# lliutianc/MPVAE-1

Measured on AMD Instinct MI355X. Metric: probit MC label-samples/sec (B×n_sample×L) at 1/2/4/8 GPU; ELBO rel-err, higher is better.
Workload: dtype f32; 1 GPU; c4: compute_loss fwd+bwd, B=512, L=1024, z=1024, n_sample=4096 (4096/GPU), philox noise on device; global_batch=512, n_sample=4096, label_dim=1024, z_dim=1024, parallelism=n_sample-sharded x1, gemm=f16x3

## Files before the change

### mpvae-1_amd/csrc/probit_fwd.hip

```cpp
#include <cstdlib>
#include <cstring>

#include "abi_util.h"
#include "mpv_common.h"

namespace mpv {

int launch_sum_slabs(const float* in, int64_t nslab, int64_t n, void* out, int out_dtype,
                     hipStream_t s);

struct FwdParams {
  const float* y;
  const float* fe;
  const float* fx;
  const float* R;
  const float* eps;
  mpv_split16 R16;
  mpv_split16 eps16;
  float* T;
  float* rowpart;
  float* colpart;
  int S, B, L, z;
  int ldT;
  int nNt, nSc, tps, nSt;
// ... 350 lines not shown
#pragma unroll
      for (int kk = 0; kk < kBK / 16; ++kk) {
        f32x4 a[TM], bb[TN];
#pragma unroll
        for (int m = 0; m < TM; ++m)
          a[m] = *reinterpret_cast<const f32x4*>(
              &As[(wm * TM * 16 + m * 16 + lr) * kLDK + kk * 16 + lg * 4]);
#pragma unroll
        for (int n = 0; n < TN; ++n)
          bb[n] = *reinterpret_cast<const f32x4*>(
              &Bs[(wn * TN * 16 + n * 16 + lr) * kLDK + kk * 16 + lg * 4]);
#pragma unroll
        for (int j = 0; j < 4; ++j)
#pragma unroll
          for (int m = 0; m < TM; ++m)
#pragma unroll
            for (int n = 0; n < TN; ++n)
              acc[m][n] = __builtin_amdgcn_mfma_f32_16x16x4f32(a[m][j], bb[n][j], acc[m][n], 0, 0, 0);
      }
      __syncthreads();
      if (kc + 1 < nK) {
        store_tiles();
        __syncthreads();
      }
    }
    if constexpr (PREDICT)
      fwd_tile_epilogue_predict<WM, WN, TM, TN>(p, ln, acc, 1.0f, b, s0, s0, nt);
    else
      fwd_tile_epilogue<WM, WN, TM, TN>(p, ln, acc, 1.0f, b, s0, s0, nt, smem);
  }
  fwd_colsum_epilogue<WM, WN, TM, TN, PREDICT>(p, ln, b, sc, n0, smem);
}

constexpr int kKC = 32;
constexpr int kRowB = 128;
constexpr int kFwdRing = 2;
constexpr int kFwd16Threads = 512;

template <int BM>
MPV_DEV int fwd_tile_s0(int st, int S) {
  return S >= BM ? min(st * BM, S - BM) : 0;
}

template <int BM, int BN, int NW>
struct Fwd16Dma {
  static constexpr int GA = BM / 8, GB = BN / 8;
  static constexpr int JA = (GA + NW - 1) / NW, JB = (GB + NW - 1) / NW;
  const char* a_base;
  const char* b_base;
  uint32_t offa[JA], offb[JB];
  int tile, kc;
  int wid;

  MPV_DEV void init(const FwdParams& p, int t0, int b, int n0, int wid_, int lane) {
    wid = wid_;
    const int64_t lda = p.eps16.ld, ldb = p.R16.ld;
    const int prow = lane >> 3, u_lds = lane & 7;
    b_base = reinterpret_cast<const char*>(p.R16.data + (int64_t)n0 * ldb);
#pragma unroll
    for (int j = 0; j < JA; ++j) {
      const int r = (wid + j * NW) * 8 + prow;
      offa[j] = (uint32_t)((int64_t)min(r, p.S - 1) * lda * 2) +
                (uint32_t)((u_lds ^ ((r >> 1) & 7)) * 16);
    }
#pragma unroll
    for (int j = 0; j < JB; ++j) {
      const int r = (wid + j * NW) * 8 + prow;
      offb[j] = (uint32_t)(r * ldb * 2) + (uint32_t)((u_lds ^ ((r >> 1) & 7)) * 16);
    }
    tile = t0;
    kc = 0;
    set_tile(p, b);
  }

  MPV_DEV void set_tile(const FwdParams& p, int b) {
    const int64_t o = ((int64_t)b * p.S + fwd_tile_s0<BM>(tile, p.S)) * p.eps16.ld;
    a_base = reinterpret_cast<const char*>(p.eps16.data + o);
  }

  MPV_DEV static void piece(const char* base, uint32_t off, char* dst) {
    lds_dma16(base, off, lds_addr(dst));
  }

  MPV_DEV void issue(const FwdParams& p, char* dst, int tile_end, int nK, int b) {
    if (tile >= tile_end) return;
    const int kb = kc * kRowB;
#pragma unroll
    for (int j = 0; j < JA; ++j) {
      const int pc = wid + j * NW;
      if (GA % NW == 0 || pc < GA) piece(a_base + kb, offa[j], dst + pc * 1024);
    }
#pragma unroll
    for (int j = 0; j < JB; ++j) {
      const int pc = wid + j * NW;
      if (GB % NW == 0 || pc < GB) piece(b_base + kb, offb[j], dst + BM * kRowB + pc * 1024);
    }
    if (++kc == nK) {
      kc = 0;
      if (++tile < tile_end) set_tile(p, b);
    }
  }
};

template <int BM, int BN, int NW>
struct Fwd16DmaLin {
  static constexpr int GA = BM / 8, GB = BN / 8;
  static constexpr int JA = GA / NW, JB = GB / NW;
  static_assert(GA % NW == 0 && GB % NW == 0, "pieces split evenly over the DMA waves");
  const char* a_base;
  const char* b_base;
  int64_t a_step, b_step;
  uint32_t offa, offb;
  int tile, kc, wid;

  MPV_DEV void init(const FwdParams& p, int t0, int b, int n0, int wid_, int lane) {
    wid = wid_;
    const int64_t lda = p.eps16.ld, ldb = p.R16.ld;
    const int prow = lane >> 3, u_lds = lane & 7;
    a_step = (int64_t)NW * 8 * lda * 2;
    b_step = (int64_t)NW * 8 * ldb * 2;
    b_base = reinterpret_cast<const char*>(p.R16.data + ((int64_t)n0 + wid * 8) * ldb);
    offa = (uint32_t)(prow * lda * 2) + (uint32_t)((u_lds ^ (((wid * 8 + prow) >> 1) & 7)) * 16);
    offb = (uint32_t)(prow * ldb * 2) + (uint32_t)((u_lds ^ (((wid * 8 + prow) >> 1) & 7)) * 16);
    tile = t0;
    kc = 0;
    set_tile(p, b);
  }
  MPV_DEV void set_tile(const FwdParams& p, int b) {
    const int64_t o = ((int64_t)b * p.S + fwd_tile_s0<BM>(tile, p.S) + wid * 8) * p.eps16.ld;
    a_base = reinterpret_cast<const char*>(p.eps16.data + o);
  }
  MPV_DEV void issue(const FwdParams& p, char* dst, int tile_end, int nK, int b) {
    if (tile >= tile_end) return;
    const int kb = kc * kRowB;
#pragma unroll
    for (int j = 0; j < JA; ++j)
      lds_dma16(a_base + kb + j * a_step, offa, lds_addr(dst + (wid + j * NW) * 1024));
#pragma unroll
    for (int j = 0; j < JB; ++j)
      lds_dma16(b_base + kb + j * b_step, offb, lds_addr(dst + BM * kRowB + (wid + j * NW) * 1024));
    if (++kc == nK) {
      kc = 0;
      if (++tile < tile_end) set_tile(p, b);
    }
  }
};

struct Fwd16tTile48x256 {
  static constexpr int WL = 1, WS = 8, TL = 3, TSA = kFwd48BM / 128, TSB = TSA;
  static constexpr int BM = kFwd48BM, BN = 48, LDS_MIN = 82 * 1024;
  using Dma = Fwd16Dma<BM, BN, 4>;
  static constexpr int CQ = 1, EPI_BLOCKS = kEpiSampleBlocks, EPI_PART = 0;
  static constexpr bool RED_IN_RING = false, AHEAD = false;
};
struct Fwd16tTile96x128 {
  static constexpr int WL = 2, WS = 4, TL = 3, TSA = 2, TSB = 2;
  static constexpr int BM = 128, BN = 96, LDS_MIN = 0;
  using Dma = Fwd16Dma<BM, BN, 4>;
  static constexpr int CQ = 1, EPI_BLOCKS = kEpiSampleBlocks, EPI_PART = 0;
  static constexpr bool RED_IN_RING = false, AHEAD = false;
};
struct Fwd16aTile128x128 {
  static constexpr int WL = 4, WS = 2, TL = 2, TSA = 5, TSB = 3;
  static constexpr int BM = 128, BN = 128, LDS_MIN = 0;
  using Dma = Fwd16Dma<BM, BN, 4>;
  static constexpr int CQ = 1, EPI_BLOCKS = kEpiSampleBlocks, EPI_PART = 0;
  static constexpr bool RED_IN_RING = false, AHEAD = false;
};
struct Fwd16aTile256x128 {
  static constexpr int WL = 4, WS = 2, TL = 4, TSA = 5, TSB = 3;
  static constexpr int BM = 128, BN = 256, LDS_MIN = 0;
  using Dma = Fwd16Dma<BM, BN, 4>;
  static constexpr int CQ = 1, EPI_BLOCKS = kEpiSampleBlocks, EPI_PART = 0;
  static constexpr bool RED_IN_RING = false, AHEAD = false;
};
struct Fwd16bTile256x256 {
  static constexpr int WL = 4, WS = 2, TL = 4, TSA = kFwdBA, TSB = 16 - kFwdBA;
  static constexpr int BM = 256, BN = 256, LDS_MIN = 0;
  using Dma = Fwd16DmaLin<BM, BN, 4>;
  static constexpr int CQ = kFwdBCQ, EPI_BLOCKS = kFwdBEpi, EPI_PART = kFwdBPart;
  static constexpr bool RED_IN_RING = true, AHEAD = true;
};

template <int TL, int TS>
struct FragT {
  s16x8 rh[TL], rl[TL], eh[TS], el[TS];
};

template <int TL, int TS, int BM>
MPV_DEV void fwd16t_read(FragT<TL, TS>& f, const char* base, int wl, int sbo, int lr, int coh,
                         int col) {
#pragma unroll
  for (int m = 0; m < TL; ++m) {
    const int off = (BM + (wl * TL + m) * 16 + lr) * kRowB;
    f.rh[m] = *reinterpret_cast<const s16x8*>(base + off + coh);
    f.rl[m] = *reinterpret_cast<const s16x8*>(base + off + col);
  }
#pragma unroll
  for (int n = 0; n < TS; ++n) {
    const int off = ((sbo + n) * 16 + lr) * kRowB;
    f.eh[n] = *reinterpret_cast<const s16x8*>(base + off + coh);
    f.el[n] = *reinterpret_cast<const s16x8*>(base + off + col);
  }
}

template <int TL, int TS>
MPV_DEV void fwd16t_mfma(f32x4 (&acc)[TL][TS], const FragT<TL, TS>& f) {
#pragma unroll
  for (int m = 0; m < TL; ++m)
#pragma unroll
    for (int n = 0; n < TS; ++n)
      acc[m][n] = __builtin_amdgcn_mfma_f32_16x16x32_f16(as_f16x8(f.rh[m]), as_f16x8(f.eh[n]),
                                                         acc[m][n], 0, 0, 0);
#pragma unroll
  for (int m = 0; m < TL; ++m)
#pragma unroll
    for (int n = 0; n < TS; ++n)
      acc[m][n] = __builtin_amdgcn_mfma_f32_16x16x32_f16(as_f16x8(f.rh[m]), as_f16x8(f.el[n]),
                                                         acc[m][n], 0, 0, 0);
#pragma unroll
  for (int m = 0; m < TL; ++m)
#pragma unroll
    for (int n = 0; n < TS; ++n)
      acc[m][n] = __builtin_amdgcn_mfma_f32_16x16x32_f16(as_f16x8(f.rl[m]), as_f16x8(f.eh[n]),
                                                         acc[m][n], 0, 0, 0);
}

template <int H>
MPV_DEV f32x2 pk_fma_bc(f32x2 a, f32x2 b, f32x2 c) {
  f32x2 d;
  if (H == 0)
    asm("v_pk_fma_f32 %0, %1, %2, %3 op_sel_hi:[1,0,0]" : "=v"(d) : "v"(a), "v"(b), "v"(c));
  else
    asm("v_pk_fma_f32 %0, %1, %2, %3 op_sel:[0,1,1] op_sel_hi:[1,1,1]"
        : "=v"(d) : "v"(a), "v"(b), "v"(c));
  return d;
}
template <int H>
MPV_DEV void pk_fma2_acc_bc(f32x2 p, f32x2 q, f32x2 r, f32x2& sp, f32x2& sn) {
  if (H == 0)
    asm("s_nop 0\n\tv_pk_fma_f32 %0, %2, %4, %0 op_sel_hi:[0,1,1]\n\t"
        "v_pk_fma_f32 %1, %3, %4, %1 op_sel_hi:[0,1,1]"
        : "+v"(sp), "+v"(sn) : "v"(p), "v"(q), "v"(r));
  else
    asm("s_nop 0\n\tv_pk_fma_f32 %0, %2, %4, %0 op_sel:[1,0,0] op_sel_hi:[1,1,1]\n\t"
        "v_pk_fma_f32 %1, %3, %4, %1 op_sel:[1,0,0] op_sel_hi:[1,1,1]"
        : "+v"(sp), "+v"(sn) : "v"(p), "v"(q), "v"(r));
}

template <int BN>
MPV_DEV bool fwd_tile_soft(const FwdParams& p, int b, int n0, int nthreads) {
  bool my_soft = false;
  for (int i = threadIdx.x; i < BN; i += nthreads) {
    const int l = n0 + i;
    if (l < p.L) {
      const float yv = p.y[(int64_t)b * p.L + l];
      my_soft |= !(yv == 0.0f || yv == 1.0f);
    }
  }
  return __builtin_amdgcn_readfirstlane(__syncthreads_or(my_soft)) != 0;
}

struct Fwd16Ctx {
  int b, sc, nt, n0;
  int wid, wl, ws;
  int lr, lg;
  int coh, col;
  float scale;
  int nK;
  int t_begin, t_end;
  bool soft_any;
  float* cacc;
  const float* cols;
};

template <class Tile, bool PREDICT = false>
MPV_DEV Fwd16Ctx fwd16_ctx(const FwdParams& p, float* cacc, float* cols) {
  constexpr int WL = Tile::WL, BN = Tile::BN,
                CACC = Tile::WS * Tile::CQ * BN * (PREDICT ? 1 : 2);
  Fwd16Ctx c;
  int g;
  decode_block(blockIdx.x, p.B * p.nSc, p.nNt, g, c.nt);
  c.b = g / p.nSc, c.sc = g % p.nSc;
  c.n0 = c.nt * BN;
  const int tid = threadIdx.x, lane = tid & 63;
  c.wid = __builtin_amdgcn_readfirstlane(tid >> 6);
  c.wl = c.wid % WL, c.ws = c.wid / WL;
  c.lr = lane & 15, c.lg = lane >> 4;
  c.scale = 1.0f / (*p.eps16.scale * *p.R16.scale);
  c.nK = (p.z + kKC - 1) / kKC;
  const int sw = (c.lr >> 1) & 7;
  c.coh = (c.lg ^ sw) << 4, c.col = ((4 + c.lg) ^ sw) << 4;
  c.t_begin = c.sc * p.tps, c.t_end = min(p.nSt, (c.sc + 1) * p.tps);
  if constexpr (PREDICT)
    fwd_cols_stage_predict<BN>(cols, p, c.b, c.n0, kFwd16Threads);
  else
    fwd_cols_stage_t<BN>(cols, p, c.b, c.n0, kFwd16Threads);
  for (int i = tid; i < CACC; i += kFwd16Threads) cacc[i] = 0.0f;
  if constexpr (PREDICT)
    c.soft_any = false;
  else
    c.soft_any = fwd_tile_soft<BN>(p, c.b, c.n0, kFwd16Threads);
  c.cacc = cacc, c.cols = cols;
  return c;
}

template <class Tile, int TS, bool FIRST = true, bool LAST = true>
MPV_DEV void fwd_tile_epilogue_t(const FwdParams& p, const Fwd16Ctx c, f32x4 (&acc)[Tile::TL][TS],
                                 int s0, int s_own, int sbo, float* red) {
  constexpr int WL = Tile::WL, TL = Tile::TL, BM = Tile::BM, BN = Tile::BN, NT = kFwd16Threads;
  const int tid = threadIdx.x, lr = c.lr, lg = c.lg;
  const int wid = tid >> 6, wl = wid % WL, ws = wid / WL;
  if constexpr (Tile::TSA == Tile::TSB) {
    static_assert(TS == Tile::TSA, "the even-split tiles run the epilogue whole");
    sbo = ws * TS;
  }
  const int S = p.S, B = p.B, L = p.L, b = c.b, nt = c.nt, n0 = nt * BN;
  const float scale = c.scale;
  float* cacc = c.cacc;
  const float* cols = c.cols;
  f32x2 sl[TS], sp[TS], sn[TS];
#pragma unroll
  for (int n = 0; n < TS; ++n) sl[n] = sp[n] = sn[n] = splat2(0.0f);
#pragma unroll
  for (int m = 0; m < TL; ++m)
#pragma unroll
    for (int n = 0; n < TS; ++n) acc[m][n] = acc[m][n] * scale;
  const bool t_plain = s0 + sbo * 16 >= s_own && s0 + (sbo + TS) * 16 <= S && n0 + BN <= L;
#pragma unroll 1
  for (int m = 0; m < TL; ++m) {
    f32x4 am[TS];
#pragma unroll
    for (int n = 0; n < TS; ++n) am[n] = acc[0][n];
#pragma unroll
    for (int mm = 0; mm + 1 < TL; ++mm)
#pragma unroll
      for (int n = 0; n < TS; ++n) acc[mm][n] = acc[mm + 1][n];
    const int lb = (wl * TL + m) * 16 + lg * 4;
    if (((m + __builtin_amdgcn_readfirstlane(wid / (NT / 128))) & 1) != 0)
      __builtin_amdgcn_s_setprio(1);
    else
      __builtin_amdgcn_s_setprio(0);
    if (p.T != nullptr && t_plain) {
#pragma unroll
      for (int n = 0; n < TS; ++n) {
        const int s = s0 + (sbo + n) * 16 + lr;
        *reinterpret_cast<f32x4*>(p.T + ((int64_t)b * S + s) * p.ldT + n0 + lb) = am[n];
      }
    } else if (p.T != nullptr) {
#pragma unroll
      for (int n = 0; n < TS; ++n) {
        const int s = s0 + (sbo + n) * 16 + lr;
        if (s >= s_own && s < S) {
          float* row = p.T + ((int64_t)b * S + s) * p.ldT + n0;
          if (n0 + lb < L) {
            *reinterpret_cast<f32x4*>(row + lb) = am[n];
          } else {
#pragma unroll
            for (int i = 0; i < 4; ++i)
              if (n0 + lb + i < L) row[lb + i] = am[n][i];
          }
        }
      }
    }
    const f32x4 pa = *reinterpret_cast<const f32x4*>(cols + 2 * lb);
    const f32x4 pb = *reinterpret_cast<const f32x4*>(cols + 2 * lb + 4);
    const f32x2 fex[4] = {f32x2{pa[0], pa[1]}, f32x2{pa[2], pa[3]}, f32x2{pb[0], pb[1]},
                          f32x2{pb[2], pb[3]}};
    const f32x4 y4 = *reinterpret_cast<const f32x4*>(cols + 2 * BN + lb);
    const f32x4 qa = *reinterpret_cast<const f32x4*>(cols + kCqa * BN + lb);
    const f32x4 qb = *reinterpret_cast<const f32x4*>(cols + kCqb * BN + lb);
    const f32x4 sga = *reinterpret_cast<const f32x4*>(cols + kCsga * BN + lb);
    const f32x4 sgb = *reinterpret_cast<const f32x4*>(cols + kCsgb * BN + lb);
    const f32x4 wpos = *reinterpret_cast<const f32x4*>(cols + kCwpos * BN + lb);
    const f32x4 wneg = *reinterpret_cast<const f32x4*>(cols + kCwneg * BN + lb);
    const f32x2 qa2[2] = {f32x2{qa[0], qa[1]}, f32x2{qa[2], qa[3]}};
    const f32x2 qb2[2] = {f32x2{qb[0], qb[1]}, f32x2{qb[2], qb[3]}};
    const f32x2 sga2[2] = {f32x2{sga[0], sga[1]}, f32x2{sga[2], sga[3]}};
    const f32x2 sgb2[2] = {f32x2{sgb[0], sgb[1]}, f32x2{sgb[2], sgb[3]}};
    const f32x2 wpos2[2] = {f32x2{wpos[0], wpos[1]}, f32x2{wpos[2], wpos[3]}};
    const f32x2 wneg2[2] = {f32x2{wneg[0], wneg[1]}, f32x2{wneg[2], wneg[3]}};
    f32x2 ce[4] = {splat2(0.0f), splat2(0.0f), splat2(0.0f), splat2(0.0f)};
#pragma unroll
    for (int n = 0; n < TS; ++n) {
      const int s = s0 + (sbo + n) * 16 + lr;
      const float wr = (s >= s_own && s < S) ? 1.0f : 0.0f;
      const f32x4 t4 = am[n];
      f32x2 zq[4], w4[4];
#pragma unroll
      for (int i = 0; i < 4; ++i) zq[i] = pk_fma(splat2(t4[i]), splat2(kZq), fex[i]);
      probit_w2xN_zq<4>(zq, w4);
      f32x2 E4[4];
      {
#pragma clang fp contract(off)
#pragma unroll
        for (int i = 0; i < 4; ++i) E4[i] = w4[i] * kEh + splat2(kC0);
      }
      f32x2 q[4], r[4];
#pragma unroll
      for (int i = 0; i < 4; ++i) {
        q[i] = (i & 1) ? pk_fma_bc<1>(E4[i], qa2[i >> 1], qb2[i >> 1])
                       : pk_fma_bc<0>(E4[i], qa2[i >> 1], qb2[i >> 1]);
        const f32x2 a = (i & 1) ? pk_fma_bc<1>(E4[i], sga2[i >> 1], sgb2[i >> 1])
                                : pk_fma_bc<0>(E4[i], sga2[i >> 1], sgb2[i >> 1]);
        r[i] = f32x2{__builtin_amdgcn_exp2f(a.x), __builtin_amdgcn_exp2f(a.y)};
      }
      const f32x2 q4 = (q[0] * q[1]) * (q[2] * q[3]);
      f32x2 lp = f32x2{__builtin_amdgcn_logf(q4.x), __builtin_amdgcn_logf(q4.y)};
      if (c.soft_any) {
#pragma unroll
        for (int i = 0; i < 4; ++i) {
          const float y = y4[i];
          if (n0 + lb + i < L && !(y == 0.0f || y == 1.0f)) {
            const f32x2 E = E4[i];
            lp.x += y * __builtin_amdgcn_logf(E.x) + (1.0f - y) * __builtin_amdgcn_logf(1.0f - E.x);
            lp.y += y * __builtin_amdgcn_logf(E.y) + (1.0f - y) * __builtin_amdgcn_logf(1.0f - E.y);
          }
        }
      }
      sl[n] = sl[n] + lp;
#pragma unroll
      for (int i = 0; i < 4; ++i) {
        if (i & 1)
          pk_fma2_acc_bc<1>(wpos2[i >> 1], wneg2[i >> 1], r[i], sp[n], sn[n]);
        else
          pk_fma2_acc_bc<0>(wpos2[i >> 1], wneg2[i >> 1], r[i], sp[n], sn[n]);
        ce[i] = pk_fma(splat2(wr), E4[i], ce[i]);
      }
      if ((n + 1) % Tile::EPI_BLOCKS == 0) __builtin_amdgcn_sched_barrier(0);
    }
    float cs[8];
#pragma unroll
    for (int i = 0; i < 4; ++i) {
      cs[2 * i] = ce[i].x;
      cs[2 * i + 1] = ce[i].y;
    }
    if (Tile::CQ == 4) {
#pragma unroll
      for (int j = 0; j < 8; ++j) cs[j] = dpp_f<0x111>(cs[j]) + cs[j];
#pragma unroll
      for (int j = 0; j < 8; ++j) cs[j] = dpp_f<0x112>(cs[j]) + cs[j];
      if ((lr & 3) == 3) {
#pragma unroll
        for (int i = 0; i < 4; ++i) {
          float* c = cacc + ((ws * 4 + (lr >> 2)) * BN + lb + i) * 2;
          c[0] += cs[2 * i];
          c[1] += cs[2 * i + 1];
        }
      }
    } else {
      row16_sum_to_lane15_n<8>(cs);
      if (lr == 15) {
#pragma unroll
        for (int i = 0; i < 4; ++i) {
          float* c = cacc + (ws * BN + lb + i) * 2;
          c[0] += cs[2 * i];
          c[1] += cs[2 * i + 1];
        }
      }
    }
    __builtin_amdgcn_sched_barrier(0);
  }
  __builtin_amdgcn_sched_barrier(0);
  asm volatile("s_nop 1" ::: "memory");
  __builtin_amdgcn_sched_barrier(0);
  float v[TS * 6];
#pragma unroll
  for (int n = 0; n < TS; ++n) {
    sl[n] = sl[n] * 0.6931471805599453f;
    v[n * 6 + 0] = sl[n].x;
    v[n * 6 + 1] = sl[n].y;
    v[n * 6 + 2] = sp[n].x;
    v[n * 6 + 3] = sn[n].x;
    v[n * 6 + 4] = sp[n].y;
    v[n * 6 + 5] = sn[n].y;
  }
  sum_lanegroups_n<TS * 6>(v);
  if (Tile::RED_IN_RING && FIRST) lds_barrier();
  if (lg == 0) {
#pragma unroll
    for (int n = 0; n < TS; ++n)
#pragma unroll
      for (int k = 0; k < 6; ++k) red[(wl * BM + (sbo + n) * 16 + lr) * 6 + k] = v[n * 6 + k];
  }
  if (!LAST) return;
  lds_barrier();
  for (int r = tid; r < BM; r += NT) {
    const int s = s0 + r;
    if (s >= s_own && s < S) {
#pragma unroll
      for (int k = 0; k < 6; ++k) {
        float v = 0.0f;
#pragma unroll
        for (int w = 0; w < WL; ++w) v += red[(w * BM + r) * 6 + k];
        p.rowpart[(((int64_t)k * p.nNt + nt) * B + b) * S + s] = v;
      }
    }
  }
  lds_barrier();
}

template <class Tile, int TS>
MPV_DEV void fwd_tile_epilogue_predict_t(const FwdParams& p, const Fwd16Ctx c,
                                         f32x4 (&acc)[Tile::TL][TS], int s0, int s_own, int sbo) {
  constexpr int WL = Tile::WL, TL = Tile::TL, BN = Tile::BN, NT = kFwd16Threads;
  const int tid = threadIdx.x, lr = c.lr, lg = c.lg;
  const int wid = tid >> 6, wl = wid % WL, ws = wid / WL;
  if constexpr (Tile::TSA == Tile::TSB) {
    static_assert(TS == Tile::TSA, "the even-split tiles run the epilogue whole");
    sbo = ws * TS;
  }
  const int S = p.S;
  const float scale = c.scale;
  float* cacc = c.cacc;
  const float* cols = c.cols;
#pragma unroll
  for (int m = 0; m < TL; ++m)
#pragma unroll
    for (int n = 0; n < TS; ++n) acc[m][n] = acc[m][n] * scale;
#pragma unroll 1
  for (int m = 0; m < TL; ++m) {
    f32x4 am[TS];
#pragma unroll
    for (int n = 0; n < TS; ++n) am[n] = acc[0][n];
#pragma unroll
    for (int mm = 0; mm + 1 < TL; ++mm)
#pragma unroll
      for (int n = 0; n < TS; ++n) acc[mm][n] = acc[mm + 1][n];
    const int lb = (wl * TL + m) * 16 + lg * 4;
    if (((m + __builtin_amdgcn_readfirstlane(wid / (NT / 128))) & 1) != 0)
      __builtin_amdgcn_s_setprio(1);
    else
      __builtin_amdgcn_s_setprio(0);
    const f32x4 fx4 = *reinterpret_cast<const f32x4*>(cols + lb);
    const f32x2 fx2[2] = {f32x2{fx4[0], fx4[1]}, f32x2{fx4[2], fx4[3]}};
    f32x2 ce[2] = {splat2(0.0f), splat2(0.0f)};
#pragma unroll
    for (int n = 0; n < TS; ++n) {
      const int s = s0 + (sbo + n) * 16 + lr;
      const float wr = (s >= s_own && s < S) ? 1.0f : 0.0f;
      const f32x4 t4 = am[n];
      f32x2 zq[2], w2[2];
      zq[0] = pk_fma(f32x2{t4[0], t4[1]}, splat2(kZq), fx2[0]);
      zq[1] = pk_fma(f32x2{t4[2], t4[3]}, splat2(kZq), fx2[1]);
      probit_w2xN_zq<2>(zq, w2);
      f32x2 E2[2];
      {
#pragma clang fp contract(off)
#pragma unroll
        for (int j = 0; j < 2; ++j) E2[j] = w2[j] * kEh + splat2(kC0);
      }
#pragma unroll
      for (int j = 0; j < 2; ++j) ce[j] = pk_fma(splat2(wr), E2[j], ce[j]);
      if ((n + 1) % Tile::EPI_BLOCKS == 0) __builtin_amdgcn_sched_barrier(0);
    }
    float cs[4] = {ce[0].x, ce[0].y, ce[1].x, ce[1].y};
    if (Tile::CQ == 4) {
#pragma unroll
      for (int j = 0; j < 4; ++j) cs[j] = dpp_f<0x111>(cs[j]) + cs[j];
#pragma unroll
      for (int j = 0; j < 4; ++j) cs[j] = dpp_f<0x112>(cs[j]) + cs[j];
      if ((lr & 3) == 3) {
#pragma unroll
        for (int i = 0; i < 4; ++i) cacc[(ws * 4 + (lr >> 2)) * BN + lb + i] += cs[i];
      }
    } else {
      row16_sum_to_lane15_n<4>(cs);
      if (lr == 15) {
#pragma unroll
        for (int i = 0; i < 4; ++i) cacc[ws * BN + lb + i] += cs[i];
      }
    }
    __builtin_amdgcn_sched_barrier(0);
  }
}

template <int NSLOT, int BN, bool PREDICT = false>
MPV_DEV void fwd16t_colpart(const FwdParams& p, const float* cacc, int b, int sc, int n0) {
  lds_barrier();
  if constexpr (PREDICT) {
    for (int c = threadIdx.x; c < BN; c += kFwd16Threads) {
      const int l = n0 + c;
      if (l < p.L) {
        float x = 0.f;
#pragma unroll
        for (int w = 0; w < NSLOT; ++w) x += cacc[w * BN + c];
        p.colpart[((int64_t)sc * p.B + b) * p.L + l] = x;
      }
    }
    return;
  }
  for (int c = threadIdx.x; c < BN; c += kFwd16Threads) {
    const int l = n0 + c;
    if (l < p.L) {
      float e = 0.f, x = 0.f;
#pragma unroll
      for (int w = 0; w < NSLOT; ++w) {
        e += cacc[(w * BN + c) * 2 + 0];
        x += cacc[(w * BN + c) * 2 + 1];
      }
      p.colpart[(((int64_t)sc * 2 + 0) * p.B + b) * p.L + l] = e;
      p.colpart[(((int64_t)sc * 2 + 1) * p.B + b) * p.L + l] = x;
    }
  }
}

template <class Tile, int TSW>
MPV_DEV void fwd16_stage_ahead(f32x4 (&acc)[Tile::TL][TSW], const char* base, int wl, int sbo, int lr,
                               int coh, int col) {
  constexpr int TL = Tile::TL, BM = Tile::BM;
  s16x8 rh[TL], rl[TL];
#pragma unroll
  for (int m = 0; m < TL; ++m) {
    const int off = (BM + (wl * TL + m) * 16 + lr) * kRowB;
    rh[m] = *reinterpret_cast<const s16x8*>(base + off + coh);
    rl[m] = *reinterpret_cast<const s16x8*>(base + off + col);
  }
  s16x8 eh = *reinterpret_cast<const s16x8*>(base + (sbo * 16 + lr) * kRowB + coh);
  s16x8 el = *reinterpret_cast<const s16x8*>(base + (sbo * 16 + lr) * kRowB + col);
#pragma unroll
  for (int n = 0; n < TSW; ++n) {
    s16x8 eh2, el2;
    if (n + 1 < TSW) {
      const int off = ((sbo + n + 1) * 16 + lr) * kRowB;
      eh2 = *reinterpret_cast<const s16x8*>(base + off + coh);
      el2 = *reinterpret_cast<const s16x8*>(base + off + col);
    }
#pragma unroll
    for (int m = 0; m < TL; ++m)
      acc[m][n] = __builtin_amdgcn_mfma_f32_16x16x32_f16(as_f16x8(rh[m]), as_f16x8(eh), acc[m][n], 0, 0, 0);
#pragma unroll
    for (int m = 0; m < TL; ++m)
      acc[m][n] = __builtin_amdgcn_mfma_f32_16x16x32_f16(as_f16x8(rh[m]), as_f16x8(el), acc[m][n], 0, 0, 0);
#pragma unroll
    for (int m = 0; m < TL; ++m)
      acc[m][n] = __builtin_amdgcn_mfma_f32_16x16x32_f16(as_f16x8(rl[m]), as_f16x8(eh), acc[m][n], 0, 0, 0);
    if (n + 1 < TSW) {
      eh = eh2;
      el = el2;
    }
  }
}

template <class Tile, int TSW, int PART = 0, bool PREDICT = false>
MPV_DEV void fwd16_epilogue(const FwdParams& p, const Fwd16Ctx c, f32x4 (&acc)[Tile::TL][TSW], int s0,
                            int s_own, int sbo, float* red) {
  constexpr int NP = (Tile::EPI_PART > 0 && TSW / Tile::EPI_PART > 0) ? TSW / Tile::EPI_PART : 1;
  if constexpr (PREDICT) {
    if constexpr (NP == 1) {
      fwd_tile_epilogue_predict_t<Tile, TSW>(p, c, acc, s0, s_own, sbo);
    } else {
      constexpr int H0 = TSW / NP, H = PART + 1 < NP ? H0 : TSW - (NP - 1) * H0;
      f32x4 a[Tile::TL][H];
#pragma unroll
      for (int m = 0; m < Tile::TL; ++m)
#pragma unroll
        for (int n = 0; n < H; ++n) a[m][n] = acc[m][PART * H0 + n];
      fwd_tile_epilogue_predict_t<Tile, H>(p, c, a, s0, s_own, sbo + PART * H0);
      if constexpr (PART + 1 < NP)
        fwd16_epilogue<Tile, TSW, PART + 1, true>(p, c, acc, s0, s_own, sbo, red);
    }
  } else if constexpr (NP == 1) {
    fwd_tile_epilogue_t<Tile, TSW>(p, c, acc, s0, s_own, sbo, red);
  } else {
    constexpr int H0 = TSW / NP, H = PART + 1 < NP ? H0 : TSW - (NP - 1) * H0;
    f32x4 a[Tile::TL][H];
#pragma unroll
    for (int m = 0; m < Tile::TL; ++m)
#pragma unroll
      for (int n = 0; n < H; ++n) a[m][n] = acc[m][PART * H0 + n];
    fwd_tile_epilogue_t<Tile, H, PART == 0, PART == NP - 1>(p, c, a, s0, s_own, sbo + PART * H0, red);
    if constexpr (PART + 1 < NP) fwd16_epilogue<Tile, TSW, PART + 1>(p, c, acc, s0, s_own, sbo, red);
  }
}

template <class Tile, int TSW, bool PREDICT = false>
MPV_DEV void fwd16_tiles(const FwdParams& p, const Fwd16Ctx c, char* smem, float* red_lds,
                         typename Tile::Dma& dma, bool dmaw, int sbo) {
  constexpr int TL = Tile::TL, BM = Tile::BM;
  constexpr int STAGE = (BM + Tile::BN) * kRowB;
  int gs = 0;
  for (int st = c.t_begin; st < c.t_end; ++st) {
    const int s0 = fwd_tile_s0<BM>(st, p.S);
    f32x4 acc[TL][TSW];
#pragma unroll
    for (int m = 0; m < TL; ++m)
#pragma unroll
      for (int n = 0; n < TSW; ++n) acc[m][n] = f32x4{0.f, 0.f, 0.f, 0.f};
    for (int kc = 0; kc < c.nK; ++kc, ++gs) {
      wait_vmcnt<0>();
      asm volatile("s_waitcnt lgkmcnt(0)" ::: "memory");
      barrier_raw();
      if (dmaw) {
        dma.issue(p, smem + ((__builtin_amdgcn_readfirstlane(gs) + kFwdRing - 1) % kFwdRing) * STAGE,
                  c.t_end, c.nK, c.b);
      }
      const char* img = smem + (gs % kFwdRing) * STAGE;
      if constexpr (Tile::AHEAD) {
        fwd16_stage_ahead<Tile, TSW>(acc, img, c.wl, sbo, c.lr, c.coh, c.col);
      } else {
        FragT<TL, TSW> f;
        fwd16t_read<TL, TSW, BM>(f, img, c.wl, sbo, c.lr, c.coh, c.col);
        fwd16t_mfma<TL, TSW>(acc, f);
      }
    }
    __builtin_amdgcn_s_setprio(0);
    float* red = Tile::RED_IN_RING
                     ? reinterpret_cast<float*>(smem + ((gs + kFwdRing - 1) % kFwdRing) * STAGE)
                     : red_lds;
    fwd16_epilogue<Tile, TSW, 0, PREDICT>(p, c, acc, s0, st * BM, sbo, red);
    if (dmaw)
      __builtin_amdgcn_s_setprio(1);
    else
      __builtin_amdgcn_s_setprio(0);
  }
}

constexpr int kPredictLdsMin = 82 * 1024;
template <class Tile, bool PREDICT = false>
__global__ __launch_bounds__(kFwd16Threads, 1) void probit_fwd16_kernel(FwdParams p) {
  constexpr int WL = Tile::WL, WS = Tile::WS, TSA = Tile::TSA, TSB = Tile::TSB;
  constexpr int BM = Tile::BM, BN = Tile::BN;
  static_assert(WL * WS * 64 == kFwd16Threads && BN == WL * Tile::TL * 16 &&
                    BM == WS / 2 * (TSA + TSB) * 16 && (TSA == TSB || WS == 2),
                "the descriptor's geometry");
  constexpr int STAGE = (BM + BN) * kRowB;
  constexpr int RED = (Tile::RED_IN_RING || PREDICT) ? 0 : WL * BM * 6,
                CACC = WS * Tile::CQ * BN * (PREDICT ? 1 : 2);
  static_assert(!Tile::RED_IN_RING || WL * BM * 6 * 4 <= STAGE, "red fits one stage image");
  constexpr int LDS = kFwdRing * STAGE + (RED + CACC + (PREDICT ? 1 : kColsT) * BN) * 4;
  constexpr int LDS_MIN = (PREDICT && Tile::LDS_MIN < kPredictLdsMin) ? kPredictLdsMin : Tile::LDS_MIN;
  __shared__ __attribute__((aligned(1024))) char smem[LDS > LDS_MIN ? LDS : LDS_MIN];
  float* red = reinterpret_cast<float*>(smem + kFwdRing * STAGE);
  float* cacc = red + RED;

  const Fwd16Ctx c = fwd16_ctx<Tile, PREDICT>(p, cacc, cacc + CACC);
  const bool dmaw = c.wid >= 4;
  typename Tile::Dma dma;
  dma.init(p, c.t_begin, c.b, c.n0, c.wid % 4, threadIdx.x & 63);
  if (dmaw) {
#pragma unroll
    for (int j = 0; j < kFwdRing - 1; ++j) dma.issue(p, smem + j * STAGE, c.t_end, c.nK, c.b);
  }
  if (dmaw) __builtin_amdgcn_s_setprio(1);
  if constexpr (TSA == TSB)
    fwd16_tiles<Tile, TSA, PREDICT>(p, c, smem, red, dma, dmaw, c.ws * TSA);
  else if (c.wid < 4)
    fwd16_tiles<Tile, TSA, PREDICT>(p, c, smem, red, dma, false, 0);
  else
    fwd16_tiles<Tile, TSB, PREDICT>(p, c, smem, red, dma, true, TSA);
  fwd16t_colpart<WS * Tile::CQ, BN, PREDICT>(p, cacc, c.b, c.sc, c.n0);
}

__global__ __launch_bounds__(256) void predict_final_kernel(const float* __restrict__ part, int nSc,
                                                            int split, int64_t n,
                                                            float* __restrict__ colsum,
                                                            float* __restrict__ indiv,
                                                            float S_total, uint64_t* seed_advance) {
  if (seed_advance != nullptr && blockIdx.x == 0 && threadIdx.x == 0) *seed_advance += 1ull;
  for (int64_t i = (int64_t)blockIdx.x * blockDim.x + threadIdx.x; i < n;
       i += (int64_t)gridDim.x * blockDim.x) {
    float x;
    if (part == nullptr) {
      x = colsum[i];
    } else {
      if (split) {
        float g[16];
#pragma unroll
        for (int j = 0; j < 16; ++j) g[j] = 0.0f;
        for (int k0 = 0; k0 < nSc; k0 += 16) {
#pragma unroll
          for (int j = 0; j < 16; ++j)
            if (k0 + j < nSc) g[j] += part[(int64_t)(k0 + j) * n + i];
        }
        x = g[0];
#pragma unroll
        for (int j = 1; j < 16; ++j) x += g[j];
      } else {
        x = 0.0f;
#pragma unroll 8
        for (int k = 0; k < nSc; ++k) x += part[(int64_t)k * n + i];
      }
      colsum[i] = x;
    }
    if (indiv != nullptr) indiv[i] = x / S_total;
  }
}

constexpr int kFinalThreads = 1024;
template <class Row>
MPV_DEV void finalize_scalars(const mpv_final_args& a, int B, float S_total, Row row) {
  __shared__ float red[16 * 5];
  const int tid = threadIdx.x;
  float ne = 0.f, nx = 0.f, ce = 0.f, cx = 0.f;
  for (int b = tid; b < B; b += blockDim.x) {
    float v[6];
    row(b, v);
    ne += -logf(v[1] / S_total) - v[0];
    nx += -logf(v[3] / S_total) - v[2];
    ce += v[4];
    cx += v[5];
  }
  float kl = 0.f;
  const int64_t nd = (int64_t)B * a.d;
  auto klt = [](float lve, float lvx, float mue, float mux) {
    const float dm = mux - mue;
    return (lvx - lve) - 1.0f + expf(lve - lvx) + dm * dm / (expf(lvx) + kKlEps);
  };
  const bool vec = (nd & 3) == 0 &&
                   ((reinterpret_cast<uintptr_t>(a.fe_logvar) | reinterpret_cast<uintptr_t>(a.fx_logvar) |
                     reinterpret_cast<uintptr_t>(a.fe_mu) | reinterpret_cast<uintptr_t>(a.fx_mu)) & 15) == 0;
  if (vec) {
    for (int64_t i = 4 * (int64_t)tid; i < nd; i += 4 * (int64_t)blockDim.x) {
      const f32x4 le = *reinterpret_cast<const f32x4*>(a.fe_logvar + i);
      const f32x4 lx = *reinterpret_cast<const f32x4*>(a.fx_logvar + i);
      const f32x4 me = *reinterpret_cast<const f32x4*>(a.fe_mu + i);
      const f32x4 mx = *reinterpret_cast<const f32x4*>(a.fx_mu + i);
#pragma unroll
      for (int q = 0; q < 4; ++q) kl += klt(le[q], lx[q], me[q], mx[q]);
    }
  } else {
#pragma unroll 4
    for (int64_t i = tid; i < nd; i += blockDim.x)
      kl += klt(a.fe_logvar[i], a.fx_logvar[i], a.fe_mu[i], a.fx_mu[i]);
  }
  float r5[5] = {ne, nx, ce, cx, kl};
  block_reduce_n<5, false>(r5, red);
  ne = r5[0], nx = r5[1], ce = r5[2], cx = r5[3], kl = r5[4];
  if (tid == 0) {
    const float nll = ne / (float)B, nll_x = nx / (float)B;
    const float c = ce / (S_total * (float)B), c_x = cx / (S_total * (float)B);
    const float klv = 0.5f * kl / (float)B;
    *a.nll = nll;
    *a.nll_x = nll_x;
    *a.c = c;
    *a.c_x = c_x;
    *a.kl = klv;
    *a.total = (nll + nll_x) * a.nll_coeff + (c + c_x) * a.c_coeff + klv * kKlWeight;
  }
}

MPV_DEV void write_indiv(const mpv_final_args& a, int64_t n, int64_t i, float e, float x,
                         float S_total) {
  a.indiv_prob_label[i] = e / S_total;
  a.indiv_prob[i] = x / S_total;
  (void)n;
}

__global__ __launch_bounds__(kCombineThreads) void fwd_combine_kernel(const float* __restrict__ y,
                                                         const float* __restrict__ rowpart,
                                                         float* __restrict__ rowstat,
                                                         float* __restrict__ bstat, int S, int B,
                                                         int L, int nNt,
                                                         const float* __restrict__ colpart,
                                                         float* __restrict__ colsum, int nSc) {
  __shared__ float red[32], red2[32];
  const int b = blockIdx.x, tid = threadIdx.x;
  if (colpart != nullptr) {
// ... 405 lines not shown
```

Measured before the change: 76.63 billion label-samples/s.

## Restructure probit forward epilogue: unrolled label passes, asm stores, fused exp/FMA, zero-init MFMA

The epilogue no longer pre-scales and shifts the whole accumulator array. It scales per label group as it is consumed, processes EPI_UNROLL label groups per pass, and indexes accumulator slices in place instead of copying partial arrays. T stores go through inline global_store_dwordx4 with a scalar base, and exp2 is interleaved with the packed FMA accumulation in asm. The first K stage now feeds zero directly into the MFMA instead of zero-initialising the accumulators, and the stage-ahead LDS reads use precomputed 32-bit addresses. The aim is to cut register moves, address arithmetic and VALU stalls in the epilogue, at the cost of more register pressure and fragile hand-written asm, such as dropping an s_nop hazard guard.

New measurement: 76.64 billion label-samples/s (median of 2 runs). Within noise of the previous version (+0.0%).

```diff
diff --git a/mpvae-1_amd/csrc/probit_fwd.hip b/mpvae-1_amd/csrc/probit_fwd.hip
--- a/mpvae-1_amd/csrc/probit_fwd.hip
+++ b/mpvae-1_amd/csrc/probit_fwd.hip
@@ -526,6 +526,7 @@
   using Dma = Fwd16Dma<BM, BN, 4>;
   static constexpr int CQ = 1, EPI_BLOCKS = kEpiSampleBlocks, EPI_PART = 0;
   static constexpr bool RED_IN_RING = false, AHEAD = false;
+  static constexpr int EPI_UNROLL = 1;
 };
 struct Fwd16tTile96x128 {
   static constexpr int WL = 2, WS = 4, TL = 3, TSA = 2, TSB = 2;
@@ -533,6 +534,7 @@
   using Dma = Fwd16Dma<BM, BN, 4>;
   static constexpr int CQ = 1, EPI_BLOCKS = kEpiSampleBlocks, EPI_PART = 0;
   static constexpr bool RED_IN_RING = false, AHEAD = false;
+  static constexpr int EPI_UNROLL = TL;
 };
 struct Fwd16aTile128x128 {
   static constexpr int WL = 4, WS = 2, TL = 2, TSA = 5, TSB = 3;
@@ -540,6 +542,7 @@
   using Dma = Fwd16Dma<BM, BN, 4>;
   static constexpr int CQ = 1, EPI_BLOCKS = kEpiSampleBlocks, EPI_PART = 0;
   static constexpr bool RED_IN_RING = false, AHEAD = false;
+  static constexpr int EPI_UNROLL = TL;
 };
 struct Fwd16aTile256x128 {
   static constexpr int WL = 4, WS = 2, TL = 4, TSA = 5, TSB = 3;
@@ -547,6 +550,7 @@
   using Dma = Fwd16Dma<BM, BN, 4>;
   static constexpr int CQ = 1, EPI_BLOCKS = kEpiSampleBlocks, EPI_PART = 0;
   static constexpr bool RED_IN_RING = false, AHEAD = false;
+  static constexpr int EPI_UNROLL = TL;
 };
 struct Fwd16bTile256x256 {
   static constexpr int WL = 4, WS = 2, TL = 4, TSA = kFwdBA, TSB = 16 - kFwdBA;
@@ -554,6 +558,7 @@
   using Dma = Fwd16DmaLin<BM, BN, 4>;
   static constexpr int CQ = kFwdBCQ, EPI_BLOCKS = kFwdBEpi, EPI_PART = kFwdBPart;
   static constexpr bool RED_IN_RING = true, AHEAD = true;
+  static constexpr int EPI_UNROLL = TL;
 };
 
 template <int TL, int TS>
@@ -578,14 +583,14 @@
   }
 }
 
-template <int TL, int TS>
+template <int TL, int TS, bool ZERO>
 MPV_DEV void fwd16t_mfma(f32x4 (&acc)[TL][TS], const FragT<TL, TS>& f) {
 #pragma unroll
   for (int m = 0; m < TL; ++m)
 #pragma unroll
     for (int n = 0; n < TS; ++n)
-      acc[m][n] = __builtin_amdgcn_mfma_f32_16x16x32_f16(as_f16x8(f.rh[m]), as_f16x8(f.eh[n]),
-                                                         acc[m][n], 0, 0, 0);
+      acc[m][n] = __builtin_amdgcn_mfma_f32_16x16x32_f16(
+          as_f16x8(f.rh[m]), as_f16x8(f.eh[n]), ZERO ? f32x4{0.f, 0.f, 0.f, 0.f} : acc[m][n], 0, 0, 0);
 #pragma unroll
   for (int m = 0; m < TL; ++m)
 #pragma unroll
@@ -610,14 +615,36 @@
         : "=v"(d) : "v"(a), "v"(b), "v"(c));
   return d;
 }
+MPV_DEV f32x2 pk_exp2_asm(f32x2 a) {
+  float x, y;
+  asm("v_exp_f32 %0, %2\n\tv_exp_f32 %1, %3" : "=&v"(x), "=&v"(y) : "v"(a.x), "v"(a.y));
+  return f32x2{x, y};
+}
+template <int H>
+MPV_DEV f32x2 pk_exp2_fma2_acc_bc(f32x2 a, f32x2 p, f32x2 q, f32x2 r, f32x2& sp, f32x2& sn) {
+  float x, y;
+  if (H == 0)
+    asm("v_exp_f32 %0, %4\n\tv_exp_f32 %1, %5\n\t"
+        "v_pk_fma_f32 %2, %6, %8, %2 op_sel_hi:[0,1,1]\n\t"
+        "v_pk_fma_f32 %3, %7, %8, %3 op_sel_hi:[0,1,1]"
+        : "=&v"(x), "=&v"(y), "+v"(sp), "+v"(sn)
+        : "v"(a.x), "v"(a.y), "v"(p), "v"(q), "v"(r));
+  else
+    asm("v_exp_f32 %0, %4\n\tv_exp_f32 %1, %5\n\t"
+        "v_pk_fma_f32 %2, %6, %8, %2 op_sel:[1,0,0] op_sel_hi:[1,1,1]\n\t"
+        "v_pk_fma_f32 %3, %7, %8, %3 op_sel:[1,0,0] op_sel_hi:[1,1,1]"
+        : "=&v"(x), "=&v"(y), "+v"(sp), "+v"(sn)
+        : "v"(a.x), "v"(a.y), "v"(p), "v"(q), "v"(r));
+  return f32x2{x, y};
+}
 template <int H>
 MPV_DEV void pk_fma2_acc_bc(f32x2 p, f32x2 q, f32x2 r, f32x2& sp, f32x2& sn) {
   if (H == 0)
-    asm("s_nop 0\n\tv_pk_fma_f32 %0, %2, %4, %0 op_sel_hi:[0,1,1]\n\t"
+    asm("v_pk_fma_f32 %0, %2, %4, %0 op_sel_hi:[0,1,1]\n\t"
         "v_pk_fma_f32 %1, %3, %4, %1 op_sel_hi:[0,1,1]"
         : "+v"(sp), "+v"(sn) : "v"(p), "v"(q), "v"(r));
   else
-    asm("s_nop 0\n\tv_pk_fma_f32 %0, %2, %4, %0 op_sel:[1,0,0] op_sel_hi:[1,1,1]\n\t"
+    asm("v_pk_fma_f32 %0, %2, %4, %0 op_sel:[1,0,0] op_sel_hi:[1,1,1]\n\t"
         "v_pk_fma_f32 %1, %3, %4, %1 op_sel:[1,0,0] op_sel_hi:[1,1,1]"
         : "+v"(sp), "+v"(sn) : "v"(p), "v"(q), "v"(r));
 }
@@ -679,9 +706,10 @@
   return c;
 }
 
-template <class Tile, int TS, bool FIRST = true, bool LAST = true>
-MPV_DEV void fwd_tile_epilogue_t(const FwdParams& p, const Fwd16Ctx c, f32x4 (&acc)[Tile::TL][TS],
+template <class Tile, int TSW, int N0, int TS, bool FIRST = true, bool LAST = true>
+MPV_DEV void fwd_tile_epilogue_t(const FwdParams& p, const Fwd16Ctx c, f32x4 (&acc)[Tile::TL][TSW],
                                  int s0, int s_own, int sbo, float* red) {
+  static_assert(N0 + TS <= TSW, "the call's sample blocks lie in the wave's tile");
   constexpr int WL = Tile::WL, TL = Tile::TL, BM = Tile::BM, BN = Tile::BN, NT = kFwd16Threads;
   const int tid = threadIdx.x, lr = c.lr, lg = c.lg;
   const int wid = tid >> 6, wl = wid % WL, ws = wid / WL;
@@ -696,31 +724,37 @@
   f32x2 sl[TS], sp[TS], sn[TS];
 #pragma unroll
   for (int n = 0; n < TS; ++n) sl[n] = sp[n] = sn[n] = splat2(0.0f);
-#pragma unroll
-  for (int m = 0; m < TL; ++m)
-#pragma unroll
-    for (int n = 0; n < TS; ++n) acc[m][n] = acc[m][n] * scale;
   const bool t_plain = s0 + sbo * 16 >= s_own && s0 + (sbo + TS) * 16 <= S && n0 + BN <= L;
+  const uint64_t ta = reinterpret_cast<uint64_t>(p.T) +
+                      4u * (uint64_t)(((int64_t)b * S + s0 + sbo * 16) * p.ldT + n0);
+  const uint64_t tbase =
+      ((uint64_t)(uint32_t)__builtin_amdgcn_readfirstlane((uint32_t)(ta >> 32)) << 32) |
+      (uint64_t)(uint32_t)__builtin_amdgcn_readfirstlane((uint32_t)ta);
+  const uint64_t tstep = 64u * (uint64_t)p.ldT;
+  const uint32_t trow = 4u * (uint32_t)(lr * p.ldT);
+  constexpr int U = Tile::EPI_UNROLL;
+  static_assert(TL % U == 0, "whole passes of U label groups");
 #pragma unroll 1
-  for (int m = 0; m < TL; ++m) {
+  for (int m0 = 0; m0 < TL; m0 += U) {
+#pragma unroll
+  for (int u = 0; u < U; ++u) {
+    const int m = m0 + u;
     f32x4 am[TS];
 #pragma unroll
-    for (int n = 0; n < TS; ++n) am[n] = acc[0][n];
-#pragma unroll
-    for (int mm = 0; mm + 1 < TL; ++mm)
-#pragma unroll
-      for (int n = 0; n < TS; ++n) acc[mm][n] = acc[mm + 1][n];
-    const int lb = (wl * TL + m) * 16 + lg * 4;
+    for (int n = 0; n < TS; ++n) am[n] = acc[u][N0 + n] * scale;
+    int lb = (wl * TL + m) * 16 + lg * 4;
+    asm volatile("" : "+v"(lb));
     if (((m + __builtin_amdgcn_readfirstlane(wid / (NT / 128))) & 1) != 0)
       __builtin_amdgcn_s_setprio(1);
     else
       __builtin_amdgcn_s_setprio(0);
     if (p.T != nullptr && t_plain) {
-#pragma unroll
-      for (int n = 0; n < TS; ++n) {
-        const int s = s0 + (sbo + n) * 16 + lr;
-        *reinterpret_cast<f32x4*>(p.T + ((int64_t)b * S + s) * p.ldT + n0 + lb) = am[n];
-      }
+      const uint32_t toff = trow + (uint32_t)lb * 4u;
+#pragma unroll
+      for (int n = 0; n < TS; ++n)
+        asm volatile("global_store_dwordx4 %0, %1, %2"
+                     :
+                     : "v"(toff), "v"(am[n]), "s"(tbase + (uint64_t)n * tstep));
     } else if (p.T != nullptr) {
 #pragma unroll
       for (int n = 0; n < TS; ++n) {
@@ -770,14 +804,13 @@
 #pragma unroll
         for (int i = 0; i < 4; ++i) E4[i] = w4[i] * kEh + splat2(kC0);
       }
-      f32x2 q[4], r[4];
+      f32x2 q[4], ra[4];
 #pragma unroll
       for (int i = 0; i < 4; ++i) {
         q[i] = (i & 1) ? pk_fma_bc<1>(E4[i], qa2[i >> 1], qb2[i >> 1])
                        : pk_fma_bc<0>(E4[i], qa2[i >> 1], qb2[i >> 1]);
-        const f32x2 a = (i & 1) ? pk_fma_bc<1>(E4[i], sga2[i >> 1], sgb2[i >> 1])
-                                : pk_fma_bc<0>(E4[i], sga2[i >> 1], sgb2[i >> 1]);
-        r[i] = f32x2{__builtin_amdgcn_exp2f(a.x), __builtin_amdgcn_exp2f(a.y)};
+        ra[i] = (i & 1) ? pk_fma_bc<1>(E4[i], sga2[i >> 1], sgb2[i >> 1])
+                        : pk_fma_bc<0>(E4[i], sga2[i >> 1], sgb2[i >> 1]);
       }
       const f32x2 q4 = (q[0] * q[1]) * (q[2] * q[3]);
       f32x2 lp = f32x2{__builtin_amdgcn_logf(q4.x), __builtin_amdgcn_logf(q4.y)};
@@ -793,14 +826,14 @@
         }
       }
       sl[n] = sl[n] + lp;
-#pragma unroll
-      for (int i = 0; i < 4; ++i) {
-        if (i & 1)
-          pk_fma2_acc_bc<1>(wpos2[i >> 1], wneg2[i >> 1], r[i], sp[n], sn[n]);
-        else
-          pk_fma2_acc_bc<0>(wpos2[i >> 1], wneg2[i >> 1], r[i], sp[n], sn[n]);
+      const f32x2 r0 = pk_exp2_asm(ra[0]);
+      const f32x2 r1 = pk_exp2_fma2_acc_bc<0>(ra[1], wpos2[0], wneg2[0], r0, sp[n], sn[n]);
+      const f32x2 r2 = pk_exp2_fma2_acc_bc<1>(ra[2], wpos2[0], wneg2[0], r1, sp[n], sn[n]);
+      const f32x2 r3 = pk_exp2_fma2_acc_bc<0>(ra[3], wpos2[1], wneg2[1], r2, sp[n], sn[n]);
+      pk_fma2_acc_bc<1>(wpos2[1], wneg2[1], r3, sp[n], sn[n]);
+#pragma unroll
+      for (int i = 0; i < 4; ++i)
         ce[i] = pk_fma(splat2(wr), E4[i], ce[i]);
-      }
       if ((n + 1) % Tile::EPI_BLOCKS == 0) __builtin_amdgcn_sched_barrier(0);
     }
     float cs[8];
@@ -834,6 +867,13 @@
       }
     }
     __builtin_amdgcn_sched_barrier(0);
+  }
+  if constexpr (U < TL) {
+#pragma unroll
+    for (int mm = 0; mm + U < TL; ++mm)
+#pragma unroll
+      for (int n = 0; n < TS; ++n) acc[mm][N0 + n] = acc[mm + U][N0 + n];
+  }
   }
   __builtin_amdgcn_sched_barrier(0);
   asm volatile("s_nop 1" ::: "memory");
@@ -874,9 +914,10 @@
   lds_barrier();
 }
 
-template <class Tile, int TS>
+template <class Tile, int TSW, int N0, int TS>
 MPV_DEV void fwd_tile_epilogue_predict_t(const FwdParams& p, const Fwd16Ctx c,
-                                         f32x4 (&acc)[Tile::TL][TS], int s0, int s_own, int sbo) {
+                                         f32x4 (&acc)[Tile::TL][TSW], int s0, int s_own, int sbo) {
+  static_assert(N0 + TS <= TSW, "the call's sample blocks lie in the wave's tile");
   constexpr int WL = Tile::WL, TL = Tile::TL, BN = Tile::BN, NT = kFwd16Threads;
   const int tid = threadIdx.x, lr = c.lr, lg = c.lg;
   const int wid = tid >> 6, wl = wid % WL, ws = wid / WL;
@@ -889,18 +930,10 @@
   float* cacc = c.cacc;
   const float* cols = c.cols;
 #pragma unroll
-  for (int m = 0; m < TL; ++m)
-#pragma unroll
-    for (int n = 0; n < TS; ++n) acc[m][n] = acc[m][n] * scale;
-#pragma unroll 1
   for (int m = 0; m < TL; ++m) {
     f32x4 am[TS];
 #pragma unroll
-    for (int n = 0; n < TS; ++n) am[n] = acc[0][n];
-#pragma unroll
-    for (int mm = 0; mm + 1 < TL; ++mm)
-#pragma unroll
-      for (int n = 0; n < TS; ++n) acc[mm][n] = acc[mm + 1][n];
+    for (int n = 0; n < TS; ++n) am[n] = acc[m][N0 + n] * scale;
     const int lb = (wl * TL + m) * 16 + lg * 4;
     if (((m + __builtin_amdgcn_readfirstlane(wid / (NT / 128))) & 1) != 0)
       __builtin_amdgcn_s_setprio(1);
@@ -979,30 +1012,36 @@
   }
 }
 
-template <class Tile, int TSW>
+template <class Tile, int TSW, bool ZERO>
 MPV_DEV void fwd16_stage_ahead(f32x4 (&acc)[Tile::TL][TSW], const char* base, int wl, int sbo, int lr,
                                int coh, int col) {
   constexpr int TL = Tile::TL, BM = Tile::BM;
+  const uint32_t row = lds_addr(base) + lr * kRowB;
+  uint32_t rbh = row + (BM + wl * TL * 16) * kRowB + coh, rbl = row + (BM + wl * TL * 16) * kRowB + col;
+  uint32_t ebh = row + coh, ebl = row + col;
+  asm("" : "+v"(rbh), "+v"(rbl), "+v"(ebh), "+v"(ebl));
+  auto frag = [](uint32_t b, int off) {
+    return *reinterpret_cast<const __attribute__((address_space(3))) s16x8*>((uintptr_t)(b + off));
+  };
   s16x8 rh[TL], rl[TL];
 #pragma unroll
   for (int m = 0; m < TL; ++m) {
-    const int off = (BM + (wl * TL + m) * 16 + lr) * kRowB;
-    rh[m] = *reinterpret_cast<const s16x8*>(base + off + coh);
-    rl[m] = *reinterpret_cast<const s16x8*>(base + off + col);
-  }
-  s16x8 eh = *reinterpret_cast<const s16x8*>(base + (sbo * 16 + lr) * kRowB + coh);
-  s16x8 el = *reinterpret_cast<const s16x8*>(base + (sbo * 16 + lr) * kRowB + col);
+    rh[m] = frag(rbh, m * 16 * kRowB);
+    rl[m] = frag(rbl, m * 16 * kRowB);
+  }
+  s16x8 eh = frag(ebh, sbo * 16 * kRowB);
+  s16x8 el = frag(ebl, sbo * 16 * kRowB);
 #pragma unroll
   for (int n = 0; n < TSW; ++n) {
     s16x8 eh2, el2;
     if (n + 1 < TSW) {
-      const int off = ((sbo + n + 1) * 16 + lr) * kRowB;
-      eh2 = *reinterpret_cast<const s16x8*>(base + off + coh);
-      el2 = *reinterpret_cast<const s16x8*>(base + off + col);
+      eh2 = frag(ebh, (sbo + n + 1) * 16 * kRowB);
+      el2 = frag(ebl, (sbo + n + 1) * 16 * kRowB);
     }
 #pragma unroll
     for (int m = 0; m < TL; ++m)
-      acc[m][n] = __builtin_amdgcn_mfma_f32_16x16x32_f16(as_f16x8(rh[m]), as_f16x8(eh), acc[m][n], 0, 0, 0);
+      acc[m][n] = __builtin_amdgcn_mfma_f32_16x16x32_f16(
+          as_f16x8(rh[m]), as_f16x8(eh), ZERO ? f32x4{0.f, 0.f, 0.f, 0.f} : acc[m][n], 0, 0, 0);
 #pragma unroll
     for (int m = 0; m < TL; ++m)
       acc[m][n] = __builtin_amdgcn_mfma_f32_16x16x32_f16(as_f16x8(rh[m]), as_f16x8(el), acc[m][n], 0, 0, 0);
@@ -1020,33 +1059,22 @@
 MPV_DEV void fwd16_epilogue(const FwdParams& p, const Fwd16Ctx c, f32x4 (&acc)[Tile::TL][TSW], int s0,
                             int s_own, int sbo, float* red) {
   constexpr int NP = (Tile::EPI_PART > 0 && TSW / Tile::EPI_PART > 0) ? TSW / Tile::EPI_PART : 1;
+  constexpr int H0 = TSW / NP, H = PART + 1 < NP ? H0 : TSW - (NP - 1) * H0;
   if constexpr (PREDICT) {
-    if constexpr (NP == 1) {
-      fwd_tile_epilogue_predict_t<Tile, TSW>(p, c, acc, s0, s_own, sbo);
-    } else {
-      constexpr int H0 = TSW / NP, H = PART + 1 < NP ? H0 : TSW - (NP - 1) * H0;
-      f32x4 a[Tile::TL][H];
-#pragma unroll
-      for (int m = 0; m < Tile::TL; ++m)
-#pragma unroll
-        for (int n = 0; n < H; ++n) a[m][n] = acc[m][PART * H0 + n];
-      fwd_tile_epilogue_predict_t<Tile, H>(p, c, a, s0, s_own, sbo + PART * H0);
-      if constexpr (PART + 1 < NP)
-        fwd16_epilogue<Tile, TSW, PART + 1, true>(p, c, acc, s0, s_own, sbo, red);
-    }
-  } else if constexpr (NP == 1) {
-    fwd_tile_epilogue_t<Tile, TSW>(p, c, acc, s0, s_own, sbo, red);
+    fwd_tile_epilogue_predict_t<Tile, TSW, PART * H0, H>(p, c, acc, s0, s_own, sbo + PART * H0);
+    if constexpr (PART + 1 < NP)
+      fwd16_epilogue<Tile, TSW, PART + 1, true>(p, c, acc, s0, s_own, sbo, red);
   } else {
-    constexpr int H0 = TSW / NP, H = PART + 1 < NP ? H0 : TSW - (NP - 1) * H0;
-    f32x4 a[Tile::TL][H];
-#pragma unroll
-    for (int m = 0; m < Tile::TL; ++m)
-#pragma unroll
-      for (int n = 0; n < H; ++n) a[m][n] = acc[m][PART * H0 + n];
-    fwd_tile_epilogue_t<Tile, H, PART == 0, PART == NP - 1>(p, c, a, s0, s_own, sbo + PART * H0, red);
+    fwd_tile_epilogue_t<Tile, TSW, PART * H0, H, PART == 0, PART == NP - 1>(p, c, acc, s0, s_own,
+                                                                            sbo + PART * H0, red);
     if constexpr (PART + 1 < NP) fwd16_epilogue<Tile, TSW, PART + 1>(p, c, acc, s0, s_own, sbo, red);
   }
 }
+
+template <bool V>
+struct BoolC {
+  static constexpr bool value = V;
+};
 
 template <class Tile, int TSW, bool PREDICT = false>
 MPV_DEV void fwd16_tiles(const FwdParams& p, const Fwd16Ctx c, char* smem, float* red_lds,
@@ -1057,11 +1085,7 @@
   for (int st = c.t_begin; st < c.t_end; ++st) {
     const int s0 = fwd_tile_s0<BM>(st, p.S);
     f32x4 acc[TL][TSW];
-#pragma unroll
-    for (int m = 0; m < TL; ++m)
-#pragma unroll
-      for (int n = 0; n < TSW; ++n) acc[m][n] = f32x4{0.f, 0.f, 0.f, 0.f};
-    for (int kc = 0; kc < c.nK; ++kc, ++gs) {
+    auto stage = [&](auto first) {
       wait_vmcnt<0>();
       asm volatile("s_waitcnt lgkmcnt(0)" ::: "memory");
       barrier_raw();
@@ -1071,13 +1095,16 @@
       }
       const char* img = smem + (gs % kFwdRing) * STAGE;
       if constexpr (Tile::AHEAD) {
-        fwd16_stage_ahead<Tile, TSW>(acc, img, c.wl, sbo, c.lr, c.coh, c.col);
+        fwd16_stage_ahead<Tile, TSW, decltype(first)::value>(acc, img, c.wl, sbo, c.lr, c.coh, c.col);
       } else {
         FragT<TL, TSW> f;
         fwd16t_read<TL, TSW, BM>(f, img, c.wl, sbo, c.lr, c.coh, c.col);
-        fwd16t_mfma<TL, TSW>(acc, f);
-      }
-    }
+        fwd16t_mfma<TL, TSW, decltype(first)::value>(acc, f);
+      }
+      ++gs;
+    };
+    stage(BoolC<true>{});
+    for (int kc = 1; kc < c.nK; ++kc) stage(BoolC<false>{});
     __builtin_amdgcn_s_setprio(0);
     float* red = Tile::RED_IN_RING
                      ? reinterpret_cast<float*>(smem + ((gs + kFwdRing - 1) % kFwdRing) * STAGE)
```
